# Liaoyongjian1/HC-MVS

Hardware: AMD Instinct MI355X
Metric: PatchMatch Mpix/s (1080p, 8 views, 7x7, 8 iter) (higher is better)
Workload: dtype f32; 1 GPU; batch of 32 independent units per GPU, each 1 ref x 8 src views, 1920x1080, 7x7 taps (adapthalfwin 6), 8 sweeps, it_external 0, full EstimateDepthMap (median + init score + sweeps + end pass); batch=32, exchange=none

## Files before the change

### hc-mvs_amd/csrc/hcmvs_api.cpp

```cpp
#include "../../include/hcmvs_hip.h"
#include "pm_common.h"
#include "fuse_common.h"
#include "pf_chain.h"
#include "filter_plan.h"
#include "tri_init.h"
#include "cloud_kernels.h"
#include "vis_kernels.h"
#include "dev_buf.h"

#include <cmath>
#include <cstdarg>
#include <cstdio>
#include <cstring>
#include <map>
#include <string>
#include <algorithm>
#include <chrono>
#include <vector>

using namespace hcmvs;

namespace {

constexpr int kMaxBatch = HCMVS_MAX_BATCH;
// ... 8 lines not shown
	DevBuf gra;
	DevBuf keep;
	DevBuf quads;
	double K[9], R[9], C[3];
	float *mDepth = nullptr, *mNormal = nullptr, *mConf = nullptr;
	DevBuf depthMem, normalMem, confMem;
	float dMin = 0.f, dMax = 0.f;
	DevBuf dNeighbors;
	std::vector<uint32_t> neighbors;
	const float *sDepth = nullptr, *sNormal = nullptr, *sConf = nullptr;
	bool rescaled = false;
};

}


struct hcmvs_ctx final : Reclaimer {
	int device = 0;
	hipStream_t ownStream = nullptr;
	hipStream_t stream = nullptr;
	std::string err;
	std::map<uint32_t, View> views;
	struct Slot {
		explicit Slot(Reclaimer* r) : dn(r), conf(r), tmpDepth(r), progress(r), srcSlab(r) {}
		DevBuf dn, conf, tmpDepth;
		DevBuf progress;
		DevBuf srcSlab;
	};
	std::vector<Slot> slots;
	DevBuf tmpU8{this};
	DevBuf maskStage{this};
	DevBuf sDepth{this}, sNormal{this}, sConf{this};
	DevBuf dViews{this};
	std::vector<DevView> hViews;
	DevBuf dItems{this};
	std::vector<EstConst> hItems;
	DevBuf dSpread{this};
	std::vector<SpreadView> hSpread;
	int viewspread = 0;
	bool haveSpreadStats = false;
	DevBuf sync{this};
	int sweepPerLaunch = 0;
	DevBuf evals{this};
	hipEvent_t ev[4] = {nullptr, nullptr, nullptr, nullptr};
	int lastSweeps = 0, lastSweepLaunches = 0;
	bool haveStats = false;
	int sweepLag = 1;
	int sweepSegment = -1;
// ... 291 lines not shown
	if (it == c->views.end() || !it->second.gray) return fail(c, HCMVS_ERR_INVALID, "get_view_gray: unknown view %u (or a fuse-only view)", id);
	HIPCHK(c, hipSetDevice(c->device));
	HIPCHK(c, hipMemcpyAsync(out, it->second.gray, (size_t)it->second.w * it->second.h * sizeof(float), hipMemcpyDeviceToHost, c->stream));
	HIPCHK(c, hipStreamSynchronize(c->stream));
	return HCMVS_OK;
}

int hcmvs_release_view(hcmvs_ctx* c, uint32_t id) {
	if (!c) return HCMVS_ERR_INVALID;
	auto it = c->views.find(id);
	if (it == c->views.end()) return fail(c, HCMVS_ERR_INVALID, "release_view: unknown view %u", id);
	HIPCHK(c, hipSetDevice(c->device));
	HIPCHK(c, hipStreamSynchronize(c->stream));
	c->views.erase(it);
	return HCMVS_OK;
}

static int ensure_slot(hcmvs_ctx* c, int i, size_t n, int rows) {
	while ((int)c->slots.size() <= i) c->slots.emplace_back(c);
	hcmvs_ctx::Slot& sl = c->slots[i];
	HIPCHK(c, sl.dn.reserve(n * sizeof(float4), c->stream));
	HIPCHK(c, sl.conf.reserve(n * sizeof(float), c->stream));
	HIPCHK(c, sl.tmpDepth.reserve(n * sizeof(float), c->stream));
	HIPCHK(c, sl.progress.reserve((size_t)rows * kProgressStride * sizeof(int32_t), c->stream));
	return HCMVS_OK;
}

static int ensure_gradient(hcmvs_ctx* c, View& v) {
	if (v.gra.capacity()) return HCMVS_OK;
	const int n = v.w * v.h;
	HIPCHK(c, c->tmpU8.reserve((size_t)n, c->stream));
	HIPCHK(c, v.gra.reserve((size_t)n, c->stream));
	if (v.bgr) launch_bgr_to_u8(v.bgr, c->tmpU8.get<uint8_t>(), n, c->stream);
	else launch_gray_to_u8(v.gray, c->tmpU8.get<uint8_t>(), n, c->stream);
	launch_gradient_map(c->tmpU8.get<uint8_t>(), v.gra.get<uint8_t>(), v.w, v.h, c->stream);
	HIPCHK(c, hipGetLastError());
	return HCMVS_OK;
}

static int ensure_quads(hcmvs_ctx* c, View& v) {
	if (v.quads.capacity()) return HCMVS_OK;
	HIPCHK(c, v.quads.reserve((size_t)v.w * v.h * sizeof(float4), c->stream));
	launch_quads(v.gray, v.quads.get<float4>(), v.w, v.h, c->stream);
	HIPCHK(c, hipGetLastError());
	return HCMVS_OK;
}
// ... 122 lines not shown
		HIPCHK(c, srcSlab.reserve(slab.size, c->stream));
		for (int v = 0; v < n_src; ++v) {
			const View& s = c->views.find(it.src_ids[v])->second;
			HIPCHK(c, hipMemcpyAsync(srcSlab.get() + hv[v].byteOff, s.quads.get(), (size_t)s.w * s.h * sizeof(float4), hipMemcpyDeviceToDevice, c->stream));
		}
		k.imgBase = srcSlab.get();
	}
	k.dMin = it.d_min; k.dMax = it.d_max; k.dMinSqr = sqrtf(it.d_min); k.dMaxSqr = sqrtf(it.d_max);
	k.smoothBonusDepth = 1.f - p->random_smooth_bonus;
	k.smoothBonusNormal = (1.f - p->random_smooth_bonus) * 0.96f;
	k.smoothSigmaDepth = -1.f / (2.f * (p->random_smooth_depth * p->random_smooth_depth));
	{ const float r = fd2r(p->random_smooth_normal_deg); k.smoothSigmaNormal = -1.f / (2.f * (r * r)); }
	k.angle1Range = fd2r(p->random_angle1_deg);
	k.angle2Range = fd2r(p->random_angle2_deg);
	k.thConfSmall = p->ncc_threshold_keep * 0.2f;
	k.thConfBig = p->ncc_threshold_keep * 0.4f;
	k.thConfRand = p->ncc_threshold_keep * 0.9f;
	k.thRobust = p->ncc_threshold_keep * 1.2f;
	k.thKeep = p->ncc_threshold_keep;
	k.depthRatio = p->random_depth_ratio;
	k.pfScale = 1.f - p->photometric_flow;
	k.seed = p->seed + it.seed_offset;
	k.dn = c->slots[slot].dn.get<float4>(); k.conf = c->slots[slot].conf.get<float>(); k.progress = c->slots[slot].progress.get<int32_t>();
	k.hintDepth = nullptr; k.hintNormal = nullptr; k.hintIter = -1;
	if (it.d_hint_depth && it.d_hint_normal && p->it_external == p->n_external_iters - 1) {
		k.hintDepth = it.d_hint_depth; k.hintNormal = it.d_hint_normal; k.hintIter = p->n_estimation_iters - 1;
	}
	k.keep = ref.keep.capacity() ? ref.keep.get<uint8_t>() : nullptr;
	k.spread = nullptr;
	SpreadView* hs = c->hSpread.data() + (size_t)slot * kMaxViews;
	memset(hs, 0, sizeof(SpreadView) * kMaxViews);
	if (c->viewspread && p->it_external >= 1) {
		bool any = false;
		for (int v = 0; v < n_src; ++v) {
			const View& s = c->views.find(it.src_ids[v])->second;
			if (!s.sDepth || s.rescaled) continue;
			any = true;
			hs[v].depth = s.sDepth; hs[v].normal = s.sNormal; hs[v].conf = s.sConf;
			hs[v].w = s.w; hs[v].h = s.h;
			hs[v].cx = s.K[2]; hs[v].cy = s.K[5]; hs[v].ifx = 1.0 / s.K[0]; hs[v].ify = 1.0 / s.K[4];
			double T[9];
			mat3_mul_bt(ref.R, s.R, T);
			const double dC[3] = {s.C[0] - ref.C[0], s.C[1] - ref.C[1], s.C[2] - ref.C[2]};
			hs[v].Tz[0] = T[6]; hs[v].Tz[1] = T[7]; hs[v].Tz[2] = T[8];
			hs[v].tz = ref.R[6] * dC[0] + ref.R[7] * dC[1] + ref.R[8] * dC[2];
		}
// ... 967 lines not shown
```

### hc-mvs_amd/csrc/pm_common.h

```cpp
#ifndef HCMVS_PM_COMMON_H
#define HCMVS_PM_COMMON_H

#include <hip/hip_runtime.h>
#include <stdint.h>
#include <utility>
#include "sweep_plan.h"

namespace hcmvs {

constexpr int kHalfWindow = 7;
constexpr int kMaxHalfWindow = 10;
constexpr int kBigTaps = (kMaxHalfWindow + 1) * (kMaxHalfWindow + 1);
constexpr int kBigSlots = 128;
constexpr int kMaxViews = 16;
constexpr int kMaxSlots = 32;
constexpr int kProgressStride = 16;

struct DevView {
	uint32_t byteOff;
	int32_t w, h;
	float A[9];
	float Hm[3];
};

// ... 5 lines not shown
	double cx, cy, ifx, ify;
	double Tz[3], tz;
};

struct EstConst {
	int32_t W, H, V;
	int32_t border;
	int32_t adapthalfwin, nRandomIters, itExternal, propHalfwin, propStep;
	const float* ref;
	const uint8_t* gra;
	const DevView* views;
	const char* imgBase;
	float Hr[9];
	double cx, cy, ifx, ify;
	float dMin, dMax, dMinSqr, dMaxSqr;
	float smoothBonusDepth, smoothBonusNormal, smoothSigmaDepth, smoothSigmaNormal;
	float angle1Range, angle2Range;
	float thConfSmall, thConfBig, thConfRand, thRobust, thKeep;
	float depthRatio, pfScale;
	uint32_t seed;
	float4* dn;
	float* conf;
	int32_t* progress;
	const float* hintDepth;
	const float* hintNormal;
	int32_t hintIter;
	const uint8_t* keep;
	const SpreadView* spread;
};

struct SweepSync {
	int32_t* ticket;
	int32_t* rowsDone;
	int32_t* error;
	unsigned long long* evals;
};

struct SweepArgs {
	const EstConst* dItems;
	int nItems, maxRows;
	SweepSync sync;
	int lag, affinity;
};

void launch_gray_to_u8(const float* gray, uint8_t* out, int n, hipStream_t s);
void launch_bgr_to_u8(const uint8_t* bgr, uint8_t* out, int n, hipStream_t s);
// ... 12 lines not shown
```

### hc-mvs_amd/csrc/pm_kernels.hip

```cpp
#include "pm_common.h"
#include "pm_math.h"

#include <float.h>
#include <type_traits>

namespace hcmvs {

#define HC_SQ(x) ((x) * (x))

#ifdef HCMVS_STAMPS
__device__ unsigned long long g_stamps[32];
#define STAMP_DECL unsigned long long st_last = __builtin_amdgcn_s_memtime(), st_acc[16] = {0, 0, 0, 0, 0, 0, 0, 0, 0, 0, 0, 0, 0, 0, 0, 0}; unsigned st_cnt[16] = {0, 0, 0, 0, 0, 0, 0, 0, 0, 0, 0, 0, 0, 0, 0, 0};
#define STAMP(i) { const unsigned long long t_ = __builtin_amdgcn_s_memtime(); st_acc[i] += t_ - st_last; st_last = t_; }
#define STAMP_ARGS , unsigned long long& st_last, unsigned long long (&st_acc)[16], unsigned (&st_cnt)[16]
#define STAMP_PASS , st_last, st_acc, st_cnt
#define STAMP_FLUSH if ((threadIdx.x & 63) == 0 && (threadIdx.x >> 6) == 0) { for (int i_ = 0; i_ < 16; ++i_) atomicAdd(&g_stamps[i_], st_acc[i_]); for (int i_ = 0; i_ < 16; ++i_) atomicAdd(&g_stamps[16 + i_], (unsigned long long)st_cnt[i_]); }
#define SUBMARK(name)
#define BLOCK(name, i) ++st_cnt[i];
#define BLOCKN(name, i, n) st_cnt[i] += (unsigned)(n);
#elif defined(HCMVS_MARK)
#define STAMP_DECL
#define STAMP(i) asm volatile("; HCMARK " #i);
#define SUBMARK(name) asm volatile("; HCMARK " #name);
#define BLOCK(name, i) asm volatile("; HCMARK " #name);
// ... 59 lines not shown
	                   __ATOMIC_RELAXED, HC_SCOPE);
}
__device__ __forceinline__ float load_f(const float* p) {
	return __uint_as_float(__hip_atomic_load((HC_GLOBAL uint32_t*)p, __ATOMIC_RELAXED, HC_SCOPE));
}
__device__ __forceinline__ void store_f(float* p, float v) {
	__hip_atomic_store((HC_GLOBAL uint32_t*)p, __float_as_uint(v), __ATOMIC_RELAXED, HC_SCOPE);
}

__device__ __forceinline__ float rlf(float v, int lane) {
	return __int_as_float(__builtin_amdgcn_readlane(__float_as_int(v), lane));
}
__device__ __forceinline__ int rli(int v, int lane) { return __builtin_amdgcn_readlane(v, lane); }

template <int STEP>
__device__ __forceinline__ float lane_xor(float v) {
	if (STEP == 1) return __int_as_float(__builtin_amdgcn_update_dpp(0, __float_as_int(v), 0xB1, 0xF, 0xF, false));
	if (STEP == 2) return __int_as_float(__builtin_amdgcn_update_dpp(0, __float_as_int(v), 0x4E, 0xF, 0xF, false));
	if (STEP == 4) return __int_as_float(__builtin_amdgcn_update_dpp(0, __float_as_int(v), 0x141, 0xF, 0xF, false));
	if (STEP == 8) return __int_as_float(__builtin_amdgcn_update_dpp(0, __float_as_int(v), 0x140, 0xF, 0xF, false));
	if (STEP == 16) return __int_as_float(__builtin_amdgcn_ds_swizzle(__float_as_int(v), 0x401F));
	return __shfl_xor(v, 32, 64);
}
template <int S, int STEP = 1>
__device__ __forceinline__ float group_sum(float v) {
	if constexpr (STEP < S) {
		v = v + lane_xor<STEP>(v);
		return group_sum<S, STEP * 2>(v);
	} else {
		return v;
	}
}
template <int STEP>
__device__ __forceinline__ void min2_across(float& m1, float& m2) {
	if constexpr (STEP < 64) {
		const float o1 = lane_xor<STEP>(m1), o2 = lane_xor<STEP>(m2);
		const float lo = fminf(m1, o1), hi = fmaxf(m1, o1);
		m2 = fminf(hi, fminf(m2, o2));
		m1 = lo;
		min2_across<STEP * 2>(m1, m2);
	}
}

template <int NV, int STEP = 1>
__device__ __forceinline__ void min2_group(float& m1, float& m2) {
	if constexpr (STEP < NV) {
// ... 148 lines not shown
	float curConf;
	int nx, ny;
	bool slot, sprop;
	int back;
	bool isUp;
	bool loaded;
	float4 ndn;
	float nconf;
};

__device__ __forceinline__ int patch_halfwin(const EstConst& c, float tx) { return tx > 100.f ? 5 : c.adapthalfwin; }

template <int S>
__device__ __forceinline__ void load_patch_inputs(const EstConst& c, const LaneCtx<S>& L, int x, int y, PixIn<S>& in) {
	static_assert(S == 8, "one lane layout: 8 view groups x 8 tap segments");
	gcfptr ref = (gcfptr)c.ref;
	const int a = patch_halfwin(c, in.tx);
	in.center = ref[y * c.W + x];
	const int row = L.lane >> 3, col = L.lane & 7;
	const int i = -a + 2 * (row < a ? row : a), j = -a + 2 * (col < a ? col : a);
	in.I[0] = ref[__mul24(y + i, c.W) + (x + j)];
}

template <class ST>
__device__ __forceinline__ void fill_patch_64(const EstConst& c, const LaneCtx<8>& L, int x, int y, int a, const PixIn<8>& in, Patch<8>& P, ST& st) {
	const int row = L.lane >> 3, col = L.lane & 7;
	const bool valid = row <= a && col <= a;
	const int i = -a + 2 * (row < a ? row : a), j = -a + 2 * (col < a ? col : a);
	const float sigmaColor = -1.f / (2.f * HC_SQ(0.2f));
	const float sigmaSpatial = -1.f / (2.f * (float)HC_SQ(a));
	const float I = in.I[0];
	const float wColor = HC_SQ(I - in.center) * sigmaColor;
	const float wSpatial = (float)(HC_SQ(j) + HC_SQ(i)) * sigmaSpatial;
	const float we = pm_expf(wColor + wSpatial);
	const float w = valid ? we : 0.f;
	const float swi = group_sum<64>(I * w), sw = group_sum<64>(w);
	const float tm = swi / sw;
	const float t = I - tm;
	const float tw = w * t;
	P.sumW = sw;
	P.invSumW = 1.0f / sw;
	P.normSq0 = group_sum<64>(tw * t);
	P.x = x; P.y = y; P.a = a;
	P.px0 = (float)(x - a + 2 * (L.seg < a ? L.seg : a));
	st.put_patch64(row, col, (float)(y + i), w, tw);
}
template <int S, class ST>
__device__ __forceinline__ void fill_patch_big(const EstConst& c, const LaneCtx<S>& L, int x, int y, int a, float center, Patch<S>& P, ST& st) {
	constexpr int MB = (kBigTaps + S - 1) / S;
	const int nside = a + 1, nt = nside * nside;
	gcfptr ref = (gcfptr)c.ref;
	const float sigmaColor = -1.f / (2.f * HC_SQ(0.2f));
	const float sigmaSpatial = -1.f / (2.f * (float)HC_SQ(a));
	float (*bw)[kBigSlots] = st.bw;
	float sa = 0.f, sb = 0.f;
	for (int m = 0; m < MB; ++m) {
		const int k = m * S + L.seg;
		const bool valid = k < nt;
		const int kk = valid ? k : nt - 1;
		const int row = kk / nside, col = kk - row * nside;
		const int i = -a + 2 * row, j = -a + 2 * col;
		const float I = ref[__mul24(y + i, c.W) + (x + j)];
		const float wColor = HC_SQ(I - center) * sigmaColor;
		const float wSpatial = (float)(HC_SQ(j) + HC_SQ(i)) * sigmaSpatial;
		const float we = pm_expf(wColor + wSpatial);
		const float w = valid ? we : 0.f;
		sa = fmaf(I, w, sa);
		sb = sb + w;
		bw[0][k] = (float)(x + j); bw[1][k] = (float)(y + i); bw[2][k] = w; bw[3][k] = I;
	}
	const float swi = group_sum<S>(sa), sw = group_sum<S>(sb);
	const float tm = swi / sw;
	sa = 0.f;
	for (int m = 0; m < MB; ++m) {
		const int k = m * S + L.seg;
		const float t = bw[3][k] - tm;
		const float tw = bw[2][k] * t;
		sa = fmaf(tw, t, sa);
		bw[3][k] = tw;
	}
	P.sumW = sw;
	P.invSumW = 1.0f / sw;
	P.normSq0 = group_sum<S>(sa);
	P.x = x; P.y = y; P.a = a;
	P.px0 = 0.f;
}
template <int S, bool BIG, class ST>
__device__ __forceinline__ void fill_patch(const EstConst& c, const LaneCtx<S>& L, int x, int y, const PixIn<S>& in, Patch<S>& P, ST& st) {
	const int a = patch_halfwin(c, in.tx);
	if constexpr (BIG) {
		if (a > kHalfWindow) { fill_patch_big<S>(c, L, x, y, a, in.center, P, st); return; }
	}
	fill_patch_64(c, L, x, y, a, in, P, st);
}

struct Close {
	float d, n0, n1, n2;
	float kd, k0, k1, k2;
	float X0, X1, X2, conf;
	int nx, ny;
	unsigned long long closeMask, eligMask;
};

struct PixelGeom {
	double X0x, X0y;
	float v0, v1;
	float pn0, pn1, pn2, pd;
};

__device__ __forceinline__ void make_homography(const EstConst& c, const float (&vA)[9], const float (&vHm)[3], float v0, float v1,
                                                float depth, float n0, float n1, float n2, float (&H)[9]) {
	const float nx0 = fmaf(n2, 1.0f, fmaf(n1, v1, n0 * v0));
	const float inv = 1.0f / (nx0 * depth);
	float q[3];
#pragma unroll
	for (int j = 0; j < 3; ++j) q[j] = fmaf(n2, c.Hr[6 + j], fmaf(n1, c.Hr[3 + j], n0 * c.Hr[j])) * inv;
// ... 317 lines not shown
			const float4* q = (const float4*)&pk->part[k][g][pv][0];
			const float4 a = q[0], b = q[1];
			rs[k] = ((a.x + a.y) + (a.z + a.w)) + ((b.x + b.y) + (b.z + b.w));
#endif
		}
		const float Fg = __shfl(F, g * 8, 64);
		const float s = view_score(c, rs[0], rs[1], rs[2], false, P.invSumW, P.normSq0, Fg);
		float m1 = vbase + pv < c.V ? s : __builtin_huge_valf(), m2 = __builtin_huge_valf();
		min2_group<NV>(m1, m2);
		const int k = lane - base - p0;
		const int from = (k >= 0 && k < HP ? k : 0) * NV;
		const float g1 = __shfl(m1, from, 64), g2 = __shfl(m2, from, 64);
		if (k >= 0 && k < HP && ((todo >> lane) & 1ull)) min2_merge(r1, r2, g1, g2);
	}
	SUBMARK(sc_end)
}

__device__ __forceinline__ void dir2normal(float p0, float p1, float& n0, float& n1, float& n2) {
	float s0, c0, s1, c1;
	pm_sincosf(p0, &s0, &c0);
	pm_sincosf(p1, &s1, &c1);
	n0 = c0 * s1; n1 = s0 * s1; n2 = c1;
}
__device__ __forceinline__ float random_depth(const EstConst& c, float u) {
	const float r = c.dMinSqr + (c.dMaxSqr - c.dMinSqr) * u;
	return r * r;
}
__device__ __forceinline__ void random_normal(const PixelGeom& G, float u1, float u2, float& n0, float& n1, float& n2) {
	const float p0 = fd2r(0.f) + (fd2r(180.f) - fd2r(0.f)) * u1;
	const float p1 = fd2r(90.f) + (fd2r(180.f) - fd2r(90.f)) * u2;
	dir2normal(p0, p1, n0, n1, n2);
	if (dot3(n0, n1, n2, G.v0, G.v1, 1.f) > 0.f) { n0 = -n0; n1 = -n1; n2 = -n2; }
}
__device__ __forceinline__ void correct_normal_rotate(float v0, float v1, float cosAngLen, float& n0, float& n1, float& n2) {
	const float v2 = 1.f;
	const float a0 = n1 * v2 - n2 * v1, a1 = n2 * v0 - n0 * v2, a2 = n0 * v1 - n1 * v0;
	const float vlen = sqrtf(dot3(v0, v1, v2, v0, v1, v2));
	float phi = (pm_acosf(cosAngLen / vlen) - fd2r(90.f)) * 1.01f;
	if (!(phi < -0.001f)) phi = -0.001f;
	const float wnorm = sqrtf(dot3(a0, a1, a2, a0, a1, a2));
	if (!(wnorm >= FLT_EPSILON)) return;
	const float iw = 1.f / wnorm;
	const float w0 = a0 * iw, w1 = a1 * iw, w2 = a2 * iw;
	const float O[9] = {0.f, -w2, w1, w2, 0.f, -w0, -w1, w0, 0.f};
	float sp, cp;
	pm_sincosf(phi, &sp, &cp);
// ... 15 lines not shown
__device__ __forceinline__ void correct_normal(const PixelGeom& G, float& n0, float& n1, float& n2) {
	const float cosAngLen = dot3(n0, n1, n2, G.v0, G.v1, 1.f);
	if (cosAngLen >= 0.f) correct_normal_rotate(G.v0, G.v1, cosAngLen, n0, n1, n2);
}
__device__ __forceinline__ float interpolate_pixel(const EstConst& c, const PixelGeom& G, int nx, int ny, float depth,
                                                   float n0, float n1, float n2) {
	const double p0 = n0, p1 = n1, p2 = n2, z = depth;
	const double P0 = ((double)nx - c.cx) * z * c.ifx, P1 = ((double)ny - c.cy) * z * c.ify;
	const double planeD = p0 * P0 + p1 * P1 + p2 * z;
	const float dn = (float)(planeD / (p0 * G.X0x + p1 * G.X0y + p2 * 1.0));
	return (c.dMin <= dn && dn < c.dMax) ? dn : depth;
}
__device__ __forceinline__ void init_plane(PixelGeom& G, float depth, float n0, float n1, float n2) {
	G.pn0 = n0; G.pn1 = n1; G.pn2 = n2;
	G.pd = -depth * dot3(n0, n1, n2, G.v0, G.v1, 1.f);
}
__device__ __forceinline__ void pixel_geom(const EstConst& c, int x, int y, PixelGeom& G) {
	G.X0x = ((double)x - c.cx) * c.ifx;
	G.X0y = ((double)y - c.cy) * c.ify;
	G.v0 = (float)G.X0x; G.v1 = (float)G.X0y;
	G.pn0 = G.pn1 = G.pn2 = G.pd = 0.f;
}

__device__ __forceinline__ float smooth_pass(const EstConst& c, const float (*cl)[kMaxSlots], unsigned long long closeMask,
                                             unsigned long long eligMask, int lane, float hd, float h0, float h1, float h2,
                                             float hp0, float hp1, float hp2, float hpd, int limit) {
	float F = 1.f;
	if (closeMask == 0ull) return F;
	const int nChunks = (64 - __builtin_clzll(closeMask) + 7) >> 3;
	const int j = lane & 7;
	for (int ch = 0; ch < nChunks; ++ch) {
		SUBMARK(blk_smooth_chunk)
		const int slot = ch * 8 + j;
		const float X0 = cl[0][slot], X1 = cl[1][slot], X2 = cl[2][slot];
		const float o0 = cl[3][slot], o1 = cl[4][slot], o2 = cl[5][slot];
		const float k0 = cl[6][slot], k1 = cl[7][slot], k2 = cl[8][slot];
		const bool valid = (closeMask >> slot) & 1ull;
		const bool corr = ((eligMask >> slot) & 1ull) && slot <= limit;
		const float c0 = corr ? k0 : o0, c1 = corr ? k1 : o1, c2 = corr ? k2 : o2;
		const float dist = dot3(hp0, hp1, hp2, X0, X1, X2) + hpd;
		const float fd = pm_expf(HC_SQ(dist / hd) * c.smoothSigmaDepth);
		float ca = dot3(h0, h1, h2, c0, c1, c2);
		ca = ca < -1.f ? -1.f : (ca > 1.f ? 1.f : ca);
		const float ang = pm_acosf(ca);
		const float fn = pm_expf(HC_SQ(ang) * c.smoothSigmaNormal);
		float f = (1.f - c.smoothBonusDepth * fd) * (1.f - c.smoothBonusNormal * fn);
		f = valid ? f : 1.f;
		f = f * lane_xor<1>(f);
		f = f * lane_xor<2>(f);
		f = f * lane_xor<4>(f);
		F = ch == 0 ? f : F * f;
	}
	SUBMARK(blk_smooth_end)
	return F;
}


constexpr int kHist = 16;

template <int NW>
struct RowShared {
	float sc[2][32];
	float hist[kHist][6];
	int row, item;
};

__device__ __forceinline__ int wait_progress(HC_GLOBAL int32_t* word, int need, HC_GLOBAL int32_t* err, int started = -0x7fffffff) {
#if defined(HCMVS_ABL) && HCMVS_ABL == 3
// ... 193 lines not shown
			}
		}
		float hd = 0.f, h0 = 0.f, h1 = 0.f, h2 = -1.f, hq0 = 0.f, hq1 = 0.f;
		int hlimit = 63, r0, r1;
		bool hv = false, planeOwn = true;
		if (phase == PH_PROP) {
			BLOCK(blk_gen_prop, 1)
			r0 = cb; r1 = cb + 8 * NW < nc ? cb + 8 * NW : nc;
			hd = qd; h0 = q0; h1 = q1; h2 = q2; hlimit = candSlot;
			hv = lane >= r0 && lane < r1;
		} else if (phase == PH_RAND) {
			BLOCK(blk_gen_rand, 2)
			r0 = 0; r1 = nR; planeOwn = false;
			if (lane < nR) {
				uint32_t rkr = rk;
				asm volatile("" : "+v"(rkr));
				hd = random_depth(c, rand_unit(rkr, 3u * lane));
				random_normal(G, rand_unit(rkr, 3u * lane + 1u), rand_unit(rkr, 3u * lane + 2u), h0, h1, h2);
				hv = true;
			}
		} else {
			BLOCK(blk_gen_refine, 3)
			r0 = t0; r1 = nR;
			if (lane >= t0 && lane < nR) {
				const uint32_t cbase = 64u + 3u * lane;
				hd = depth + (depthRange * scaleRange) * (2.f * rand_unit(rk, cbase) - 1.f);
				if (c.dMin <= hd && hd < c.dMax) {
					hq0 = p0 + (c.angle1Range * scaleRange) * (2.f * rand_unit(rk, cbase + 1u) - 1.f);
					hq1 = p1 + (c.angle2Range * scaleRange) * (2.f * rand_unit(rk, cbase + 2u) - 1.f);
					dir2normal(hq0, hq1, h0, h1, h2);
					hv = !(dot3(h0, h1, h2, G.v0, G.v1, 1.f) >= 0.f);
				}
			}
		}
		const unsigned long long vmask = __ballot(hv);
		STAMP(3)
		const int cnt = r1 - r0, per = (cnt + NW - 1) / NW, lo = r0 + wv * per, hi = (lo + per < r1 ? lo + per : r1);
		float best1 = __builtin_huge_valf(), best2 = __builtin_huge_valf();
		for (int base = lo; base < hi; base += 8) {
			BLOCK(blk_chunk, 4)
			const int g = base + (lane >> 3);
			const int src = g < r1 ? g : r0;
			const float gd = __shfl(hd, src, 64), g0 = __shfl(h0, src, 64), g1 = __shfl(h1, src, 64), g2 = __shfl(h2, src, 64);
			const int glimit = __shfl(hlimit, src, 64);
			const float gp0 = planeOwn ? g0 : G.pn0, gp1 = planeOwn ? g1 : G.pn1, gp2 = planeOwn ? g2 : G.pn2;
			const float gpd = planeOwn ? -gd * dot3(g0, g1, g2, G.v0, G.v1, 1.f) : G.pd;
#if defined(HCMVS_ABL) && HCMVS_ABL == 2
			const float F = 1.f + 0.f * (gd + g0 + g1 + g2 + gp0 + gp1 + gp2 + gpd + (float)glimit);
#else
			BLOCKN(blk_smooth_chunks, 10, closeMask ? (64 - __builtin_clzll(closeMask) + 7) >> 3 : 0)
			const float F = smooth_pass(c, st.pk->cl, closeMask, eligMask, lane, gd, g0, g1, g2, gp0, gp1, gp2, gpd, glimit);
#endif
			const int top = base + 8 < hi ? base + 8 : hi;
			const unsigned long long todo = vmask & ((1ull << top) - 1ull) & ~((1ull << base) - 1ull);
			STAMP(4)
			if (todo) {
				BLOCK(blk_score_chunk, 5)
				score_chunk<S, BIG, PACK>(c, L, P, st, G.v0, G.v1, F, hd, h0, h1, h2, todo, base, __builtin_ctzll(todo), best1, best2, issued);
				if constexpr (TWO) {
					unsigned again = 0;
					score_chunk<S, BIG, PACK>(c, L1, P, st, G.v0, G.v1, F, hd, h0, h1, h2, todo, base, __builtin_ctzll(todo), best1, best2, again);
				}
			}
		}
		const float mine = two_best(c, best1, best2);
		STAMP(7)
		if (hooked && !pollTaken) { pollTaken = true; if (pp.r > 0 && pp.poll > pp.known) pp.known = pp.poll; }
		const float all = share_scores<NW>(sh, par, lane, lo, hi, mine);
		STAMP(8)
		if (phase == PH_PROP) {
			BLOCK(blk_acc_prop, 6)
			for (int i = r0; i < r1; ++i) {
				BLOCK(blk_acc_prop_cand, 7)
				const float nconf = rlf(all, i);
// ... 76 lines not shown
			const bool slotV = ld && sd > 0.f;
			const double z = sd;
			const double Xc0 = ((double)cnx - sv[j].cx) * z * sv[j].ifx, Xc1 = ((double)cny - sv[j].cy) * z * sv[j].ify;
			const float zt = (float)(((sv[j].Tz[0] * Xc0 + sv[j].Tz[1] * Xc1) + sv[j].Tz[2] * z) + sv[j].tz);
			const bool open = slotV && !(scf >= c.thKeep);
			const bool hv = open && zt > 0.f;
			float k0 = sn0, k1 = sn1, k2 = sn2;
			if (hv) correct_normal(G, k0, k1, k2);
			closeMask = __ballot(slotV);
			eligMask = __ballot(hv);
			if (wv == 0) {
				spc.outside += (unsigned)__builtin_popcountll(__ballot(cand && !inMap));
				spc.dropped += (unsigned)__builtin_popcountll(__ballot(open && !hv));
			}
			if (lane < kMaxSlots) {
				cl[0][lane] = (float)Xc0; cl[1][lane] = (float)Xc1; cl[2][lane] = sd;
				cl[3][lane] = sn0; cl[4][lane] = sn1; cl[5][lane] = sn2;
				cl[6][lane] = k0; cl[7][lane] = k1; cl[8][lane] = k2;
			}
			if (eligMask == 0ull) continue;
			const int src = (lane >> 3) < 4 ? (lane >> 3) : 0;
			const float gd = __shfl(zt, src, 64), g0 = __shfl(k0, src, 64), g1 = __shfl(k1, src, 64), g2 = __shfl(k2, src, 64);
			const float gpd = -gd * dot3(g0, g1, g2, G.v0, G.v1, 1.f);
			const float F = smooth_pass(c, cl, closeMask, eligMask, lane, gd, g0, g1, g2, g0, g1, g2, gpd, src);
			float s1 = __builtin_huge_valf(), s2 = __builtin_huge_valf();
			score_chunk<S, BIG, PACK>(c, L, P, st, G.v0, G.v1, F, zt, k0, k1, k2, eligMask, 0, __builtin_ctzll(eligMask), s1, s2, issued);
			if constexpr (TWO) {
				unsigned again = 0;
				score_chunk<S, BIG, PACK>(c, L1, P, st, G.v0, G.v1, F, zt, k0, k1, k2, eligMask, 0, __builtin_ctzll(eligMask), s1, s2, again);
			}
			const float all = two_best(c, s1, s2);
			for (unsigned long long mk = eligMask; mk; mk &= mk - 1ull) {
				const int i = __builtin_ctzll(mk);
				const float nconf = rlf(all, i);
				++evals;
				if (wv == 0) ++spc.scored;
				if (conf > nconf) {
					conf = nconf; depth = rlf(zt, i); n0 = rlf(k0, i); n1 = rlf(k1, i); n2 = rlf(k2, i);
					if (wv == 0) ++spc.accepted;
				}
			}
		}
	}
	if constexpr (HINT) if (c.hintDepth && iter == c.hintIter) {
		const float hdep = as_global(c.hintDepth)[idx];
		if (hdep > 0.f) {
			float h0 = as_global(c.hintNormal)[3 * idx], h1 = as_global(c.hintNormal)[3 * idx + 1], h2 = as_global(c.hintNormal)[3 * idx + 2];
			const float hd = interpolate_pixel(c, G, x, y, hdep, h0, h1, h2);
			correct_normal(G, h0, h1, h2);
			const float hpd = -hd * dot3(h0, h1, h2, G.v0, G.v1, 1.f);
			const float F = smooth_pass(c, st.pk->cl, closeMask, eligMask, lane, hd, h0, h1, h2, h0, h1, h2, hpd, 63);
			float s1 = __builtin_huge_valf(), s2 = __builtin_huge_valf();
			score_chunk<S, BIG, PACK>(c, L, P, st, G.v0, G.v1, F, hd, h0, h1, h2, 1ull, 0, 0, s1, s2, issued);
			if constexpr (TWO) {
				unsigned again = 0;
				score_chunk<S, BIG, PACK>(c, L1, P, st, G.v0, G.v1, F, hd, h0, h1, h2, 1ull, 0, 0, s1, s2, again);
			}
			const float nconf = rlf(two_best(c, s1, s2), 0);
			++evals;
			if (conf > nconf - 0.1f) { conf = nconf; depth = hd; n0 = h0; n1 = h1; n2 = h2; }
		}
	}
	if (hooked && !pollTaken && pp.r > 0 && pp.poll > pp.known) pp.known = pp.poll;
	if (lane == 0) {
		float* hrec = sh.hist[q & (kHist - 1)];
		hrec[0] = depth; hrec[1] = n0; hrec[2] = n1; hrec[3] = n2; hrec[4] = conf;
		if (wv == NW - 1) {
			store_dn(&c.dn[idx], depth, n0, n1, n2);
			store_f(&c.conf[idx], conf);
		}
	}
	if constexpr (NW == 1) {
		pp.pendingPub = q + 1;
	} else if (wv == NW - 1) {
// ... 144 lines not shown
			first.tx = (float)pp.tx1;
			load_patch_inputs<S>(c, L, xs, y, first);
			pp.nI = first.I[0]; pp.nC = first.center;
			pp.tx2 = q0 + 1 < q1 ? uniform_byte(c.gra, y * c.W + xs + dx) : (uint8_t)0;
		}
		STAMP(9)
		for (int q = q0; q < q1 && !pp.fail; ++q) {
			const int x = rev ? c.W - 1 - bd - q : bd + q;
			STAMP(13)
			PixIn<S> in;
			in.tx = (float)pp.tx1;
			prefetch_static<S>(c, L, x, y, q, rev, pp.known >= q + 1, in);
			in.I[0] = pp.nI; in.center = pp.nC;
			if (q + 1 < q1) {
				PixIn<S> nxt;
				nxt.tx = (float)pp.tx2;
				load_patch_inputs<S>(c, L, x + dx, y, nxt);
				pp.nI = nxt.I[0]; pp.nC = nxt.center;
			}
			pp.tx1 = pp.tx2;
			if (q + 2 < q1) pp.tx2 = uniform_byte(c.gra, y * c.W + x + 2 * dx);
			uint8_t km = 1;
			if constexpr (MASK) km = uniform_byte(c.keep ? c.keep : c.gra, y * c.W + x);
			STAMP(12)
			Patch<S> P;
			fill_patch<S, BIG>(c, L, x, y, in, P, st);
			STAMP(1)
			if (pp.known < q + 1) {
				pp.known = wait_progress(pp.upWord, pp.base + q + 1, pp.err);
				if (pp.known < 0) {
					pp.fail = true;
					asm volatile("s_waitcnt vmcnt(0)" : "+v"(pp.nI), "+v"(pp.nC) :: "memory");
					break;
				}
				pp.known -= pp.base;
				prefetch_up<S>(c, in);
			}
			asm volatile("s_waitcnt vmcnt(0)" : "+v"(pp.nI), "+v"(pp.nC) :: "memory");
			STAMP(0)
			if (MASK && c.keep && km == 0) {
				if (L.lane == 0) {
					float* hrec = sh.hist[q & (kHist - 1)];
					hrec[0] = in.cur.x; hrec[1] = in.cur.y; hrec[2] = in.cur.z; hrec[3] = in.cur.w; hrec[4] = in.curConf;
					if (wv == NW - 1) __hip_atomic_store(pp.myWord, pp.base + q + 1, __ATOMIC_RELAXED, HC_SCOPE);
				}
				pp.pendingPub = 0;
				continue;
			}
			const unsigned e0 = evals;
// ... 55 lines not shown
	st.put_view(as_global(c.views) + (L.vact ? L.view : 0), L.seg);
	LaneCtx<S> L1 = L;
	RegStore<S> st1 = st;
	if constexpr (TWO) {
		lane_init<S>(c, L1, 64 / S);
		st1.put_view(as_global(c.views) + (L1.vact ? L1.view : 0), L1.seg);
	}
	const int nrows = c.H - 2 * c.border, ncols = c.W - 2 * c.border;
	const int total = nrows * ncols;
	const int wavesPerBlock = blockDim.x >> 6;
	const int gw = blockIdx.x * wavesPerBlock + (threadIdx.x >> 6), nw = gridDim.x * wavesPerBlock;
	unsigned evals = 0;
	unsigned long long taps = 0;
	const uint32_t stream0 = (uint32_t)c.itExternal * 64u;
	for (int p = gw; p < total; p += nw) {
		const int x = c.border + p % ncols, y = c.border + p / ncols;
		const int idx = y * c.W + x;
		if constexpr (MASK) if (!uniform_byte(c.keep, idx)) continue;
		const uint32_t rk = rand_key(c.seed, (uint32_t)idx, stream0);
		PixIn<S> in;
		in.tx = (float)c.gra[idx];
		load_patch_inputs<S>(c, L, x, y, in);
		Patch<S> P;
		fill_patch<S, BIG>(c, L, x, y, in, P, st);
		PixelGeom G;
		pixel_geom(c, x, y, G);
		const float4 cur = c.dn[idx];
		float d = cur.x, n0 = cur.y, n1 = cur.z, n2 = cur.w;
		if (!(c.dMin <= d && d < c.dMax)) {
			d = random_depth(c, rand_unit(rk, 0u));
			random_normal(G, rand_unit(rk, 1u), rand_unit(rk, 2u), n0, n1, n2);
		} else if (dot3(n0, n1, n2, G.v0, G.v1, 1.f) >= 0.f) {
			random_normal(G, rand_unit(rk, 1u), rand_unit(rk, 2u), n0, n1, n2);
		}
		float m1 = __builtin_huge_valf(), m2 = __builtin_huge_valf();
		score_pixel<S, BIG>(c, L, P, st, G.v0, G.v1, 1.f, d, n0, n1, n2, m1, m2);
		if constexpr (TWO) {
			st1.copy_patch(st);
			score_pixel<S, BIG>(c, L1, P, st1, G.v0, G.v1, 1.f, d, n0, n1, n2, m1, m2);
		}
		const float s = two_best(c, m1, m2);
		++evals;
		taps += (unsigned)((P.a + 1) * (P.a + 1));
		if (L.lane == 0) {
			c.dn[idx] = make_float4(d, n0, n1, n2);
			c.conf[idx] = s;
		}
	}
	if (L.lane == 0 && evals) {
		atomicAdd(evalsOut, (unsigned long long)evals);
		atomicAdd(evalsOut + 1, (unsigned long long)evals);
		atomicAdd(evalsOut + 2, taps);
	}
}

#ifdef HCMVS_COUNT
template <int S>
__global__ void probe_score_kernel(EstConst c, Patch<S> P, RegStore<S> st, float F, float d, float n0, float n1, float n2, float* out) {
	LaneCtx<S> L;
	lane_init<S>(c, L);
	float m1 = __builtin_huge_valf(), m2 = __builtin_huge_valf();
	score_pixel<S, false>(c, L, P, st, 0.1f, 0.2f, F, d, n0, n1, n2, m1, m2);
	out[threadIdx.x] = two_best(c, m1, m2);
}
template __global__ void probe_score_kernel<8>(EstConst, Patch<8>, RegStore<8>, float, float, float, float, float, float*);
__global__ void probe_smooth_kernel(EstConst c, Close C, float* out) {
	__shared__ float cl[9][kMaxSlots];
	for (int k = 0; k < 9; ++k) cl[k][threadIdx.x & 31] = out[k * 64 + threadIdx.x];
	out[threadIdx.x] = smooth_pass(c, cl, C.closeMask, C.eligMask, threadIdx.x & 63, out[0], out[1], out[2], out[3], out[4], out[5], out[6], out[7], 63);
}
template <int S>
__global__ void probe_patch_kernel(EstConst c, PixIn<S> in, Patch<S>* out, RegStore<S>* so) {
	LaneCtx<S> L;
	lane_init<S>(c, L);
	Patch<S> P;
	__shared__ float stage[3][8][8];
	RegStore<S> st;
	st.stage = stage; st.seg = L.seg;
	fill_patch<S, false>(c, L, 100, 100, in, P, st);
	out[threadIdx.x] = P;
	so[threadIdx.x] = st;
}
template __global__ void probe_patch_kernel<8>(EstConst, PixIn<8>, Patch<8>*, RegStore<8>*);
#endif

__global__ void end_kernel(EstConst c, int finalPass, float* depth, float* normal, float* conf) {
	const int n = c.W * c.H;
	for (int i = blockIdx.x * blockDim.x + threadIdx.x; i < n; i += gridDim.x * blockDim.x) {
		float4 v = c.dn[i];
		float cf = c.conf[i];
		if (finalPass && !(c.keep && !c.keep[i])) {
			if (v.x <= 0.f || cf >= c.thKeep) { v = make_float4(0.f, 0.f, 0.f, 0.f); cf = 0.f; }
			else cf = cf >= 1.f ? 0.f : 1.f - cf;
		}
		depth[i] = v.x;
		normal[3 * i] = v.y; normal[3 * i + 1] = v.z; normal[3 * i + 2] = v.w;
		conf[i] = cf;
	}
}


__global__ void gray_to_u8_kernel(const float* g, uint8_t* out, int n) {
// ... 133 lines not shown
```

### hc-mvs_amd/host/DensifyPointCloud.cpp

```cpp
#include "../../include/hcmvs_hip.h"

#include <hip/hip_runtime.h>

#include <algorithm>
#include <atomic>
#include <chrono>
#include <cmath>
#include <condition_variable>
#include <cstdint>
#include <cstdio>
#include <cstdlib>
#include <cstring>
#include <deque>
#include <fstream>
#include <map>
#include <memory>
#include <mutex>
#include <sstream>
#include <string>
#include <thread>
#include <vector>

#include <sys/stat.h>

// ... 828 lines not shown
			for (uint32_t s : images[id].srcs) needGray[(size_t)images[id].dev][s] = 1;
		}
	}

	{
		size_t maxPx = 0, allPx = 0;
		for (uint32_t id : todo) { const size_t px = (size_t)images[id].w * images[id].h; maxPx = std::max(maxPx, px); allPx += px; }
		for (int d = 0; d < nDev; ++d) {
			size_t freeB = 0, totalB = 0;
			HIPOK(hipSetDevice(devs[(size_t)d].ordinal));
			HIPOK(hipMemGetInfo(&freeB, &totalB));
			size_t ownPx = 0, grayPx = 0;
			for (uint32_t id : todo) if (images[id].dev == d) ownPx += (size_t)images[id].w * images[id].h;
			for (size_t i = 0; i < images.size(); ++i) if (images[i].valid && needGray[(size_t)d][i]) grayPx += (size_t)images[i].w * images[i].h;
			size_t resident = ownPx * (size_t)(20 + (o.restoreHypothesis ? 16 : 0)) + grayPx * (size_t)(8 + 16) + ((size_t)1 << 30);
			if (d == 0) {
				size_t maxNb = 1;
				for (uint32_t id : todo) maxNb = std::max(maxNb, std::min<size_t>(images[id].neighbors.size(), 31));
				resident += allPx * 4 + (nDev > 1 ? allPx * 20 : 0) + maxPx * (12 * maxNb + 40);
				if (o.nFilter) resident += allPx * 8 + maxPx * 8 * 8;
				if (o.fusionMode != 1) resident += (allPx * 39 > ((size_t)4 << 30) && o.fuseCount != 0) ? allPx / 5 * (31 + 3 * 8) : allPx / 2 * 31 + allPx * 8;
			}
			int batch = o.batch;
			while (batch > 1 && resident + (size_t)batch * maxPx * 24 > freeB) batch /= 2;
			if (resident + (size_t)batch * maxPx * 24 > freeB) {
				fprintf(stderr, "error: the scene does not fit device %d: %.1f GiB needed for its share (%zu of %zu images; maps, images, source footprints%s), "
				                "%.1f GiB free.  Use more devices (--devices), a coarser --resolution-level or fewer --number-views\n",
				        devs[(size_t)d].ordinal, (resident + (size_t)batch * maxPx * 24) / 1073741824.0, (size_t)std::count_if(todo.begin(), todo.end(), [&](uint32_t id) { return images[id].dev == d; }),
				        todo.size(), d == 0 ? ", the whole scene's maps, fusion tables and cloud" : "", freeB / 1073741824.0);
				return EXIT_FAILURE;
			}
			o.batch = std::min(o.batch, batch);
			if (o.verbosity > 2) printf("Device %d (context %d of %d): %.1f GiB resident + %.1f GiB per batch of %d, %.1f GiB free\n", devs[(size_t)d].ordinal, d, nDev,
			                            resident / 1073741824.0, (size_t)batch * maxPx * 24 / 1073741824.0, batch, freeB / 1073741824.0);
		}
		HIPOK(hipSetDevice(o.device));
	}

	std::vector<char> resumed(images.size(), 0);
	std::vector<uint32_t> work;
	for (uint32_t id : todo) {
		DmapFile hdr;
		if (o.resume && load_dmap(map_path(o.workdir, "/depth%04u.dmap", id), hdr, 7, true) && hdr.w == images[id].w && hdr.h == images[id].h) resumed[id] = 1;
		else { work.push_back(id); devs[(size_t)images[id].dev].work.push_back(id); }
	}
	for (uint32_t id : todo) {
		if (!resumed[id]) continue;
		ImageData& im = images[id];
		DmapFile m;
		if (!load_dmap(map_path(o.workdir, "/depth%04u.dmap", id), m, 7)) { fprintf(stderr, "error: invalid depth-map '%s'\n", map_path(o.workdir, "/depth%04u.dmap", id).c_str()); return EXIT_FAILURE; }
		const size_t n = (size_t)im.w * im.h;
		im.dMin = m.dMin; im.dMax = m.dMax;
		HIPOK(hipSetDevice(devs[(size_t)im.dev].ordinal));
		HIPOK(hipMalloc(&im.dDepth, n * 4)); HIPOK(hipMalloc(&im.dNormal, n * 12)); HIPOK(hipMalloc(&im.dConf, n * 4));
		HIPOK(hipMemcpy(im.dDepth, m.d.data(), n * 4, hipMemcpyHostToDevice)); HIPOK(hipMemcpy(im.dNormal, m.n.data(), n * 12, hipMemcpyHostToDevice));
		HIPOK(hipMemcpy(im.dConf, m.c.data(), n * 4, hipMemcpyHostToDevice));
		if (o.verbosity > 1) printf("Depth-map for image %3u loaded from '%s' (not estimated again)\n", id, map_path(o.workdir, "/depth%04u.dmap", id).c_str());
// ... 569 lines not shown
```

Baseline: 22.81 Mpix/s.

## Cache per-pixel patch statistics across sweeps and pack smooth/normal transcendental work

The init score pass now writes each pixel's patch mean, weight sum, inverse weight sum and centered norm to a new per-slot float4 buffer. The sweep kernels read these back through a scalar load instead of recomputing three 64-lane reductions per pixel per sweep. Separately, smooth_pass packs the depth and normal exponentials into mirrored half-lanes when at most 4 close slots exist, using a DPP mirror. Refinement normal generation computes sin/cos once via a permlane32 swap instead of two sincos calls. In exchange it adds 16 B per pixel of device memory (the host memory budget is raised to match), an extra global write and read, and the risk of stale stats if the window size differed between passes.

```diff
diff --git a/hc-mvs_amd/csrc/hcmvs_api.cpp b/hc-mvs_amd/csrc/hcmvs_api.cpp
--- a/hc-mvs_amd/csrc/hcmvs_api.cpp
+++ b/hc-mvs_amd/csrc/hcmvs_api.cpp
@@ -54,8 +54,9 @@
 	std::string err;
 	std::map<uint32_t, View> views;
 	struct Slot {
-		explicit Slot(Reclaimer* r) : dn(r), conf(r), tmpDepth(r), progress(r), srcSlab(r) {}
+		explicit Slot(Reclaimer* r) : dn(r), conf(r), tmpDepth(r), pstat(r), progress(r), srcSlab(r) {}
 		DevBuf dn, conf, tmpDepth;
+		DevBuf pstat;
 		DevBuf progress;
 		DevBuf srcSlab;
 	};
@@ -393,6 +394,7 @@
 	HIPCHK(c, sl.dn.reserve(n * sizeof(float4), c->stream));
 	HIPCHK(c, sl.conf.reserve(n * sizeof(float), c->stream));
 	HIPCHK(c, sl.tmpDepth.reserve(n * sizeof(float), c->stream));
+	HIPCHK(c, sl.pstat.reserve(n * sizeof(float4), c->stream));
 	HIPCHK(c, sl.progress.reserve((size_t)rows * kProgressStride * sizeof(int32_t), c->stream));
 	return HCMVS_OK;
 }
@@ -561,6 +563,7 @@
 	k.pfScale = 1.f - p->photometric_flow;
 	k.seed = p->seed + it.seed_offset;
 	k.dn = c->slots[slot].dn.get<float4>(); k.conf = c->slots[slot].conf.get<float>(); k.progress = c->slots[slot].progress.get<int32_t>();
+	k.pstat = c->slots[slot].pstat.get<float4>();
 	k.hintDepth = nullptr; k.hintNormal = nullptr; k.hintIter = -1;
 	if (it.d_hint_depth && it.d_hint_normal && p->it_external == p->n_external_iters - 1) {
 		k.hintDepth = it.d_hint_depth; k.hintNormal = it.d_hint_normal; k.hintIter = p->n_estimation_iters - 1;
diff --git a/hc-mvs_amd/csrc/pm_common.h b/hc-mvs_amd/csrc/pm_common.h
--- a/hc-mvs_amd/csrc/pm_common.h
+++ b/hc-mvs_amd/csrc/pm_common.h
@@ -51,6 +51,7 @@
 	float4* dn;
 	float* conf;
 	int32_t* progress;
+	float4* pstat;
 	const float* hintDepth;
 	const float* hintNormal;
 	int32_t hintIter;
diff --git a/hc-mvs_amd/csrc/pm_kernels.hip b/hc-mvs_amd/csrc/pm_kernels.hip
--- a/hc-mvs_amd/csrc/pm_kernels.hip
+++ b/hc-mvs_amd/csrc/pm_kernels.hip
@@ -105,6 +105,9 @@
 	if (STEP == 16) return __int_as_float(__builtin_amdgcn_ds_swizzle(__float_as_int(v), 0x401F));
 	return __shfl_xor(v, 32, 64);
 }
+__device__ __forceinline__ float half_mirror(float v) {
+	return __int_as_float(__builtin_amdgcn_update_dpp(0, __float_as_int(v), 0x141, 0xF, 0xF, false));
+}
 template <int S, int STEP = 1>
 __device__ __forceinline__ float group_sum(float v) {
 	if constexpr (STEP < S) {
@@ -299,8 +302,9 @@
 	in.I[0] = ref[__mul24(y + i, c.W) + (x + j)];
 }
 
-template <class ST>
-__device__ __forceinline__ void fill_patch_64(const EstConst& c, const LaneCtx<8>& L, int x, int y, int a, const PixIn<8>& in, Patch<8>& P, ST& st) {
+struct PatchStat { float tm, invSumW, normSq0, sumW; };
+template <bool CACHED, class ST>
+__device__ __forceinline__ void fill_patch_64(const EstConst& c, const LaneCtx<8>& L, int x, int y, int a, const PixIn<8>& in, Patch<8>& P, ST& st, PatchStat& ps) {
 	const int row = L.lane >> 3, col = L.lane & 7;
 	const bool valid = row <= a && col <= a;
 	const int i = -a + 2 * (row < a ? row : a), j = -a + 2 * (col < a ? col : a);
@@ -311,19 +315,22 @@
 	const float wSpatial = (float)(HC_SQ(j) + HC_SQ(i)) * sigmaSpatial;
 	const float we = pm_expf(wColor + wSpatial);
 	const float w = valid ? we : 0.f;
-	const float swi = group_sum<64>(I * w), sw = group_sum<64>(w);
-	const float tm = swi / sw;
-	const float t = I - tm;
+	if constexpr (!CACHED) {
+		const float swi = group_sum<64>(I * w), sw = group_sum<64>(w);
+		ps.tm = swi / sw; ps.sumW = sw; ps.invSumW = 1.0f / sw;
+	}
+	const float t = I - ps.tm;
 	const float tw = w * t;
-	P.sumW = sw;
-	P.invSumW = 1.0f / sw;
-	P.normSq0 = group_sum<64>(tw * t);
+	if constexpr (!CACHED) ps.normSq0 = group_sum<64>(tw * t);
+	P.sumW = ps.sumW;
+	P.invSumW = ps.invSumW;
+	P.normSq0 = ps.normSq0;
 	P.x = x; P.y = y; P.a = a;
 	P.px0 = (float)(x - a + 2 * (L.seg < a ? L.seg : a));
 	st.put_patch64(row, col, (float)(y + i), w, tw);
 }
 template <int S, class ST>
-__device__ __forceinline__ void fill_patch_big(const EstConst& c, const LaneCtx<S>& L, int x, int y, int a, float center, Patch<S>& P, ST& st) {
+__device__ __forceinline__ void fill_patch_big(const EstConst& c, const LaneCtx<S>& L, int x, int y, int a, float center, Patch<S>& P, ST& st, PatchStat& ps) {
 	constexpr int MB = (kBigTaps + S - 1) / S;
 	const int nside = a + 1, nt = nside * nside;
 	gcfptr ref = (gcfptr)c.ref;
@@ -361,14 +368,20 @@
 	P.normSq0 = group_sum<S>(sa);
 	P.x = x; P.y = y; P.a = a;
 	P.px0 = 0.f;
-}
-template <int S, bool BIG, class ST>
-__device__ __forceinline__ void fill_patch(const EstConst& c, const LaneCtx<S>& L, int x, int y, const PixIn<S>& in, Patch<S>& P, ST& st) {
+	ps.tm = tm; ps.invSumW = P.invSumW; ps.normSq0 = P.normSq0; ps.sumW = sw;
+}
+template <int S, bool BIG, bool CACHED, class ST>
+__device__ __forceinline__ void fill_patch(const EstConst& c, const LaneCtx<S>& L, int x, int y, const PixIn<S>& in, Patch<S>& P, ST& st, PatchStat& ps) {
 	const int a = patch_halfwin(c, in.tx);
 	if constexpr (BIG) {
-		if (a > kHalfWindow) { fill_patch_big<S>(c, L, x, y, a, in.center, P, st); return; }
-	}
-	fill_patch_64(c, L, x, y, a, in, P, st);
+		if (a > kHalfWindow) { fill_patch_big<S>(c, L, x, y, a, in.center, P, st, ps); return; }
+	}
+	fill_patch_64<CACHED>(c, L, x, y, a, in, P, st, ps);
+}
+__device__ __forceinline__ PatchStat load_patch_stat(const float4* base, int idx) {
+	typedef __attribute__((address_space(4))) const f32x4* cf4p;
+	const f32x4 v = *(cf4p)((uintptr_t)base + (uintptr_t)(unsigned)idx * sizeof(float4));
+	return {v.x, v.y, v.z, v.w};
 }
 
 struct Close {
@@ -732,6 +745,14 @@
 	pm_sincosf(p1, &s1, &c1);
 	n0 = c0 * s1; n1 = s0 * s1; n2 = c1;
 }
+__device__ __forceinline__ void dir2normal_lo32(float p0, float p1, float& n0, float& n1, float& n2) {
+	const float p = __uint_as_float(__builtin_amdgcn_permlane32_swap(__float_as_uint(p0), __float_as_uint(p1), false, false)[0]);
+	float sn, cs;
+	pm_sincosf(p, &sn, &cs);
+	const float s1 = __uint_as_float(__builtin_amdgcn_permlane32_swap(__float_as_uint(sn), __float_as_uint(sn), false, false)[1]);
+	const float c1 = __uint_as_float(__builtin_amdgcn_permlane32_swap(__float_as_uint(cs), __float_as_uint(cs), false, false)[1]);
+	n0 = cs * s1; n1 = sn * s1; n2 = c1;
+}
 __device__ __forceinline__ float random_depth(const EstConst& c, float u) {
 	const float r = c.dMinSqr + (c.dMaxSqr - c.dMinSqr) * u;
 	return r * r;
@@ -793,6 +814,7 @@
 	G.pn0 = G.pn1 = G.pn2 = G.pd = 0.f;
 }
 
+template <bool PACK4>
 __device__ __forceinline__ float smooth_pass(const EstConst& c, const float (*cl)[kMaxSlots], unsigned long long closeMask,
                                              unsigned long long eligMask, int lane, float hd, float h0, float h1, float h2,
                                              float hp0, float hp1, float hp2, float hpd, int limit) {
@@ -800,21 +822,27 @@
 	if (closeMask == 0ull) return F;
 	const int nChunks = (64 - __builtin_clzll(closeMask) + 7) >> 3;
 	const int j = lane & 7;
+	const bool packed = PACK4 && closeMask < 16ull;
+	const bool mirror = packed && j >= 4;
 	for (int ch = 0; ch < nChunks; ++ch) {
 		SUBMARK(blk_smooth_chunk)
-		const int slot = ch * 8 + j;
+		const int slot = mirror ? 7 - j : ch * 8 + j;
 		const float X0 = cl[0][slot], X1 = cl[1][slot], X2 = cl[2][slot];
 		const float o0 = cl[3][slot], o1 = cl[4][slot], o2 = cl[5][slot];
 		const float k0 = cl[6][slot], k1 = cl[7][slot], k2 = cl[8][slot];
-		const bool valid = (closeMask >> slot) & 1ull;
+		const bool valid = ((closeMask >> slot) & 1ull) && !mirror;
 		const bool corr = ((eligMask >> slot) & 1ull) && slot <= limit;
 		const float c0 = corr ? k0 : o0, c1 = corr ? k1 : o1, c2 = corr ? k2 : o2;
 		const float dist = dot3(hp0, hp1, hp2, X0, X1, X2) + hpd;
-		const float fd = pm_expf(HC_SQ(dist / hd) * c.smoothSigmaDepth);
+		const float argD = HC_SQ(dist / hd) * c.smoothSigmaDepth;
 		float ca = dot3(h0, h1, h2, c0, c1, c2);
 		ca = ca < -1.f ? -1.f : (ca > 1.f ? 1.f : ca);
 		const float ang = pm_acosf(ca);
-		const float fn = pm_expf(HC_SQ(ang) * c.smoothSigmaNormal);
+		const float argN = HC_SQ(ang) * c.smoothSigmaNormal;
+		const float fd = pm_expf(mirror ? argN : argD);
+		float fn;
+		if (packed) fn = half_mirror(fd);
+		else fn = pm_expf(argN);
 		float f = (1.f - c.smoothBonusDepth * fd) * (1.f - c.smoothBonusNormal * fn);
 		f = valid ? f : 1.f;
 		f = f * lane_xor<1>(f);
@@ -1054,13 +1082,21 @@
 		} else {
 			BLOCK(blk_gen_refine, 3)
 			r0 = t0; r1 = nR;
+			bool trial = false;
 			if (lane >= t0 && lane < nR) {
 				const uint32_t cbase = 64u + 3u * lane;
 				hd = depth + (depthRange * scaleRange) * (2.f * rand_unit(rk, cbase) - 1.f);
 				if (c.dMin <= hd && hd < c.dMax) {
 					hq0 = p0 + (c.angle1Range * scaleRange) * (2.f * rand_unit(rk, cbase + 1u) - 1.f);
 					hq1 = p1 + (c.angle2Range * scaleRange) * (2.f * rand_unit(rk, cbase + 2u) - 1.f);
-					dir2normal(hq0, hq1, h0, h1, h2);
+					trial = true;
+				}
+			}
+			{
+				float t0_, t1_, t2_;
+				dir2normal_lo32(hq0, hq1, t0_, t1_, t2_);
+				if (trial) {
+					h0 = t0_; h1 = t1_; h2 = t2_;
 					hv = !(dot3(h0, h1, h2, G.v0, G.v1, 1.f) >= 0.f);
 				}
 			}
@@ -1081,7 +1117,7 @@
 			const float F = 1.f + 0.f * (gd + g0 + g1 + g2 + gp0 + gp1 + gp2 + gpd + (float)glimit);
 #else
 			BLOCKN(blk_smooth_chunks, 10, closeMask ? (64 - __builtin_clzll(closeMask) + 7) >> 3 : 0)
-			const float F = smooth_pass(c, st.pk->cl, closeMask, eligMask, lane, gd, g0, g1, g2, gp0, gp1, gp2, gpd, glimit);
+			const float F = smooth_pass<!BIG>(c, st.pk->cl, closeMask, eligMask, lane, gd, g0, g1, g2, gp0, gp1, gp2, gpd, glimit);
 #endif
 			const int top = base + 8 < hi ? base + 8 : hi;
 			const unsigned long long todo = vmask & ((1ull << top) - 1ull) & ~((1ull << base) - 1ull);
@@ -1204,7 +1240,7 @@
 			const int src = (lane >> 3) < 4 ? (lane >> 3) : 0;
 			const float gd = __shfl(zt, src, 64), g0 = __shfl(k0, src, 64), g1 = __shfl(k1, src, 64), g2 = __shfl(k2, src, 64);
 			const float gpd = -gd * dot3(g0, g1, g2, G.v0, G.v1, 1.f);
-			const float F = smooth_pass(c, cl, closeMask, eligMask, lane, gd, g0, g1, g2, g0, g1, g2, gpd, src);
+			const float F = smooth_pass<!BIG>(c, cl, closeMask, eligMask, lane, gd, g0, g1, g2, g0, g1, g2, gpd, src);
 			float s1 = __builtin_huge_valf(), s2 = __builtin_huge_valf();
 			score_chunk<S, BIG, PACK>(c, L, P, st, G.v0, G.v1, F, zt, k0, k1, k2, eligMask, 0, __builtin_ctzll(eligMask), s1, s2, issued);
 			if constexpr (TWO) {
@@ -1231,7 +1267,7 @@
 			const float hd = interpolate_pixel(c, G, x, y, hdep, h0, h1, h2);
 			correct_normal(G, h0, h1, h2);
 			const float hpd = -hd * dot3(h0, h1, h2, G.v0, G.v1, 1.f);
-			const float F = smooth_pass(c, st.pk->cl, closeMask, eligMask, lane, hd, h0, h1, h2, h0, h1, h2, hpd, 63);
+			const float F = smooth_pass<!BIG>(c, st.pk->cl, closeMask, eligMask, lane, hd, h0, h1, h2, h0, h1, h2, hpd, 63);
 			float s1 = __builtin_huge_valf(), s2 = __builtin_huge_valf();
 			score_chunk<S, BIG, PACK>(c, L, P, st, G.v0, G.v1, F, hd, h0, h1, h2, 1ull, 0, 0, s1, s2, issued);
 			if constexpr (TWO) {
@@ -1422,9 +1458,10 @@
 			if (q + 2 < q1) pp.tx2 = uniform_byte(c.gra, y * c.W + x + 2 * dx);
 			uint8_t km = 1;
 			if constexpr (MASK) km = uniform_byte(c.keep ? c.keep : c.gra, y * c.W + x);
+			PatchStat ps = load_patch_stat(c.pstat, y * c.W + x);
 			STAMP(12)
 			Patch<S> P;
-			fill_patch<S, BIG>(c, L, x, y, in, P, st);
+			fill_patch<S, BIG, true>(c, L, x, y, in, P, st, ps);
 			STAMP(1)
 			if (pp.known < q + 1) {
 				pp.known = wait_progress(pp.upWord, pp.base + q + 1, pp.err);
@@ -1526,7 +1563,9 @@
 		in.tx = (float)c.gra[idx];
 		load_patch_inputs<S>(c, L, x, y, in);
 		Patch<S> P;
-		fill_patch<S, BIG>(c, L, x, y, in, P, st);
+		PatchStat ps;
+		fill_patch<S, BIG, false>(c, L, x, y, in, P, st, ps);
+		if (L.lane == 0) c.pstat[idx] = make_float4(ps.tm, ps.invSumW, ps.normSq0, ps.sumW);
 		PixelGeom G;
 		pixel_geom(c, x, y, G);
 		const float4 cur = c.dn[idx];
@@ -1571,7 +1610,7 @@
 __global__ void probe_smooth_kernel(EstConst c, Close C, float* out) {
 	__shared__ float cl[9][kMaxSlots];
 	for (int k = 0; k < 9; ++k) cl[k][threadIdx.x & 31] = out[k * 64 + threadIdx.x];
-	out[threadIdx.x] = smooth_pass(c, cl, C.closeMask, C.eligMask, threadIdx.x & 63, out[0], out[1], out[2], out[3], out[4], out[5], out[6], out[7], 63);
+	out[threadIdx.x] = smooth_pass<true>(c, cl, C.closeMask, C.eligMask, threadIdx.x & 63, out[0], out[1], out[2], out[3], out[4], out[5], out[6], out[7], 63);
 }
 template <int S>
 __global__ void probe_patch_kernel(EstConst c, PixIn<S> in, Patch<S>* out, RegStore<S>* so) {
@@ -1581,7 +1620,8 @@
 	__shared__ float stage[3][8][8];
 	RegStore<S> st;
 	st.stage = stage; st.seg = L.seg;
-	fill_patch<S, false>(c, L, 100, 100, in, P, st);
+	PatchStat ps;
+	fill_patch<S, false, false>(c, L, 100, 100, in, P, st, ps);
 	out[threadIdx.x] = P;
 	so[threadIdx.x] = st;
 }
diff --git a/hc-mvs_amd/host/DensifyPointCloud.cpp b/hc-mvs_amd/host/DensifyPointCloud.cpp
--- a/hc-mvs_amd/host/DensifyPointCloud.cpp
+++ b/hc-mvs_amd/host/DensifyPointCloud.cpp
@@ -874,17 +874,17 @@
 				if (o.fusionMode != 1) resident += (allPx * 39 > ((size_t)4 << 30) && o.fuseCount != 0) ? allPx / 5 * (31 + 3 * 8) : allPx / 2 * 31 + allPx * 8;
 			}
 			int batch = o.batch;
-			while (batch > 1 && resident + (size_t)batch * maxPx * 24 > freeB) batch /= 2;
-			if (resident + (size_t)batch * maxPx * 24 > freeB) {
+			while (batch > 1 && resident + (size_t)batch * maxPx * 40 > freeB) batch /= 2;
+			if (resident + (size_t)batch * maxPx * 40 > freeB) {
 				fprintf(stderr, "error: the scene does not fit device %d: %.1f GiB needed for its share (%zu of %zu images; maps, images, source footprints%s), "
 				                "%.1f GiB free.  Use more devices (--devices), a coarser --resolution-level or fewer --number-views\n",
-				        devs[(size_t)d].ordinal, (resident + (size_t)batch * maxPx * 24) / 1073741824.0, (size_t)std::count_if(todo.begin(), todo.end(), [&](uint32_t id) { return images[id].dev == d; }),
+				        devs[(size_t)d].ordinal, (resident + (size_t)batch * maxPx * 40) / 1073741824.0, (size_t)std::count_if(todo.begin(), todo.end(), [&](uint32_t id) { return images[id].dev == d; }),
 				        todo.size(), d == 0 ? ", the whole scene's maps, fusion tables and cloud" : "", freeB / 1073741824.0);
 				return EXIT_FAILURE;
 			}
 			o.batch = std::min(o.batch, batch);
 			if (o.verbosity > 2) printf("Device %d (context %d of %d): %.1f GiB resident + %.1f GiB per batch of %d, %.1f GiB free\n", devs[(size_t)d].ordinal, d, nDev,
-			                            resident / 1073741824.0, (size_t)batch * maxPx * 24 / 1073741824.0, batch, freeB / 1073741824.0);
+			                            resident / 1073741824.0, (size_t)batch * maxPx * 40 / 1073741824.0, batch, freeB / 1073741824.0);
 		}
 		HIPOK(hipSetDevice(o.device));
 	}
```

Result: no change. 22.90 Mpix/s, median of 6 (+0.4%).
